# cvjena/ITAL

Hardware: AMD Instinct MI355X
Metric: MI-scored candidates/sec per fetch_unlabelled(k) round (higher is better)
Workload: dtype f64; 1 GPU; USPS-shaped synthetic 9298x256, k=4, perfect user, full 2^t enumeration, fetch_unlabelled + update per step; n=9298, d=256, k=4, parallelism=candidate rows sharded over 1 GPU(s), 1 record all-gather per greedy step

## Files before the change

include/ital_hip.h:

```cpp
#ifndef ITAL_HIP_H
#define ITAL_HIP_H

#include <stdint.h>

#ifdef __cplusplus
extern "C" {
#endif

typedef struct ihipStream_t* hipStream_t;

#define ITAL_MAX_T 8
#define ITAL_REC_HEADER 10
#define ITAL_JUMP_BITS 48
#define ITAL_GENERIC_MAX_DIM 20
#define ITAL_GENERIC_MAX_REL 16
#define ITAL_GENERIC_MAX_CALLS (1 << 22)
#define ITAL_TOPK_MAX 4096
#define ITAL_ROUND_MAX_CAND (1 << 21)

const char* ital_version(void);
const char* ital_last_error(void);
int64_t ital_launch_count(void);


int ital_row_norms(const double* X, int64_t n, int ldx, double* xnorm, hipStream_t stream);

int ital_rbf_cols(const double* X, const double* xnorm, int64_t n, int ldx, const double* Xs, const double* sn,
                  int c, double var, double length_scale, double* out, int64_t ldo, hipStream_t stream);

int ital_cross_cov_cols(const double* X, const double* xnorm, int64_t n, int ldx, const double* Xs,
                        const double* sn, int c, const double* W, int ldw, const double* V, int64_t ldv, int m,
                        double var, double length_scale, double* out, int64_t ldo, hipStream_t stream);

int ital_chol_append(const double* XT, const double* XTn, int ldx, double* L, int ldl, double* alpha,
                     const double* ynew, int m, int c, double var, double length_scale, double noise, int* status,
                     hipStream_t stream);

typedef struct ital_label_batch {
    int c;
    int slot[16];
    double y[16];
} ital_label_batch;
int ital_stage_labelled(const double* rows, int ldx, ital_label_batch lb, double* XT_dst, double* XTn_dst, double* y_dst,
                        hipStream_t stream);

typedef struct ital_append_desc {
    const double* rows;
    int ldx;
    ital_label_batch lb;
    const double* X;
    const double* xnorm;
    int64_t n;
    double* XT;
    double* XTn;
    double* L;
    int ldl;
    double* alpha;
    double* ybuf;
    double* V;
    int64_t ldv;
    int m;
    double var, length_scale, noise;
    double* mu;
    double* s2;
    int* status;
} ital_append_desc;
int ital_gp_append(const ital_append_desc* a, hipStream_t stream);

int ital_whiten_append(const double* X, const double* xnorm, int64_t n, int ldx, const double* Xnew,
                       const double* snew, int c, const double* L21, int ldw, const double* L22,
                       const double* alpha_new, double* V, int64_t ldv, int m, double var, double length_scale,
                       double* mu, double* s2, hipStream_t stream);

int ital_predict(const double* Xt, int64_t nt, int ldx, const double* XT, const double* XTn, int m, const double* L,
                 int ldl, const double* alpha, double var, double length_scale, double* mean, double* pvar, double* xtn,
                 double* Vt, int64_t ldvt, int clamp, hipStream_t stream);

int ital_topk(const double* v, int64_t n, int64_t index_offset, int k, double* out_vals, int64_t* out_idx, void* work,
              hipStream_t stream);
int64_t ital_topk_workspace(void);

int ital_mvn_seed(int state[6]);
int ital_mvn_draws_per_call(int n);
int ital_mvn_advance(int state[6], int64_t n_draws);
int ital_mvn_round_seeds(int state[6], int64_t n_cand, int k, int seeds[][6]);
int ital_mvn_tables(int t, long long* jump, long long* jumppat, double* vk);
int ital_mvn_generic_tables(int nmax, long long* jump1, double* vk_all);

// ... 233 lines not shown
```

ital_amd/_fast_round.py:

```python
import collections
import ctypes
import time

import numpy as np
import torch

from . import _lib, mvn_stream, sharding
from ._batch import (Scored, ensure_step_buffers, fill_score_desc, fill_score_select, lattice_label, lattice_tables)
from ._lib import check
from .gp import _ptr, _stream
from .retrieval_base import UnseenList

PREPARED, COMPACT, UPLOAD = "prepared", "compact", "upload"

DeviceList = collections.namedtuple("DeviceList", "buffers unseen version picks n_loc")


class Prepared(collections.namedtuple("Prepared", "desc slot k n n_loc m begin cur state_before state_after draws events sig")):
    __slots__ = ()

    def matches(self, k, n, m, stream_state, signature):
        return (self.k == k and self.n == n and self.m == m and self.state_before == tuple(stream_state)
                and self.sig == signature)

# ... 203 lines not shown

    def _download(self):
        L, k, hc = self.L, self.k, self.L.host_clock
        if hc is not None:
            hc["enqueue_s"] += time.perf_counter() - self.t_call
        host = L._download(self.rb.b["ret"], "the picks of the round", L._step_estimate_s(k, self.n_loc)).tolist()
        if hc is not None:
            hc["t_download"] = time.perf_counter()
        keep = self.keep
        L.last_scores = [keep[t, :self.n_loc] for t in range(k)] if keep is not None else []
        return host[:k], host[self.rb.b["kmax"]]

    def _finish(self, ret, status, saved_stream):
        L, gp, c = self.L, self.gp, self.candidates
        if status & 8:
            raise RuntimeError("ital_amd: the candidate list kept on the device lost track of the host's (internal error)")
        if status & 6:
            gp.status.bitwise_and_(~6)
            self.stream.state, self.stream.draws = saved_stream
            return L._fetch_generic(self.k, c.array() if self.listed else c)
        if status:
            gp.check_status(status)
        ret = [int(i) for i in ret]
        L._last_batch = (self.rb.b, list(ret))
        if self.listed:
            self.rb.device_list = DeviceList(self.rb, c, c.version, ret, self.n_loc)
        return ret
```

ital_amd/_lib.py:

```python
import ctypes
import os

HERE = os.path.dirname(os.path.abspath(__file__))
LIB_PATH = os.environ.get("ITAL_HIP_LIB", os.path.join(HERE, "libital_hip.so"))

c_void_p, c_int, c_int64, c_double = ctypes.c_void_p, ctypes.c_int, ctypes.c_int64, ctypes.c_double

ITAL_MAX_T = 8
ITAL_REC_HEADER = 10
ITAL_JUMP_BITS = 48
ITAL_GENERIC_MAX_DIM = 20
ITAL_GENERIC_MAX_REL = 16
ITAL_GENERIC_MAX_CALLS = 1 << 22
ITAL_TOPK_MAX = 4096
ITAL_ROUND_MAX_CAND = 1 << 21


class ItalBatch(ctypes.Structure):
    _fields_ = [("kmax", c_int), ("ldx", c_int), ("ldw", c_int), ("bidx", c_void_p), ("bgpos", c_void_p),
                ("bsort", c_void_p), ("bmu", c_void_p), ("sig", c_void_p), ("XB", c_void_p), ("XBn", c_void_p),
                ("VB", c_void_p)]


class ItalLabelBatch(ctypes.Structure):
    _fields_ = [("c", c_int), ("slot", c_int * 16), ("y", c_double * 16)]


class ItalAppendDesc(ctypes.Structure):
    _fields_ = [("rows", c_void_p), ("ldx", c_int), ("lb", ItalLabelBatch), ("X", c_void_p), ("xnorm", c_void_p), ("n", c_int64),
                ("XT", c_void_p), ("XTn", c_void_p), ("L", c_void_p), ("ldl", c_int), ("alpha", c_void_p), ("ybuf", c_void_p),
                ("V", c_void_p), ("ldv", c_int64), ("m", c_int), ("var", c_double), ("length_scale", c_double),
                ("noise", c_double), ("mu", c_void_p), ("s2", c_void_p), ("status", c_void_p)]


class ItalScoreDesc(ctypes.Structure):
    _fields_ = [("t", c_int), ("n_cand", c_int64), ("cand", c_void_p), ("alive", c_void_p), ("mu", c_void_p),
                ("s2", c_void_p), ("C", c_void_p), ("ldc", c_int64), ("row_offset", c_int64),
                ("pos_offset", c_int64), ("gpos", c_void_p), ("batch", ItalBatch), ("noise", c_double), ("eps", c_double),
                ("label_mode", c_int), ("mi", c_void_p), ("seed", c_int * 6), ("jump", c_void_p), ("jumppat", c_void_p),
                ("vk", c_void_p), ("status", c_void_p), ("work", c_void_p), ("work_doubles", c_int64), ("ev_start", c_void_p),
                ("ev_stop", c_void_p), ("sel_X", c_void_p), ("sel_xnorm", c_void_p), ("sel_ldx", c_int), ("sel_V", c_void_p),
                ("sel_ldv", c_int64), ("sel_m", c_int), ("sel_ldw", c_int), ("sel_rank", c_int), ("sel_record", c_void_p),
                ("sel_ret", c_void_p), ("sel_parts", c_void_p), ("sel_parts_len", c_int64), ("sel_counter", c_void_p)]


EXCHANGE_FN = ctypes.CFUNCTYPE(c_int, c_void_p, c_void_p, c_void_p, c_int, c_void_p)


class ItalRoundDesc(ctypes.Structure):
    _fields_ = [("k", c_int), ("step", ItalScoreDesc), ("seeds", (c_int * 6) * (ITAL_MAX_T + 1)),
                ("jump", c_void_p * (ITAL_MAX_T + 1)), ("jumppat", c_void_p * (ITAL_MAX_T + 1)),
                ("vk", c_void_p * (ITAL_MAX_T + 1)), ("ev_start", c_void_p * (ITAL_MAX_T + 1)),
                ("ev_stop", c_void_p * (ITAL_MAX_T + 1)), ("n_rows", c_int64), ("var", c_double), ("length_scale", c_double),
                ("mi_keep", c_void_p), ("begin", c_int), ("cand_prev", c_void_p), ("n_prev", c_int64),
                ("world", c_int), ("records_all", c_void_p), ("nccl_comm", c_void_p), ("exchange", EXCHANGE_FN),
# ... 29 lines not shown

class ItalNpLegacyState(ctypes.Structure):
    _fields_ = [("key", ctypes.c_uint32 * 624), ("pos", ctypes.c_int32), ("has_gauss", ctypes.c_int32), ("gauss", c_double)]


SIGNATURES = {
    "ital_version": (ctypes.c_char_p, []),
    "ital_mvn_seed": (c_int, [ctypes.POINTER(c_int)]),
    "ital_mvn_draws_per_call": (c_int, [c_int]),
    "ital_mvn_advance": (c_int, [ctypes.POINTER(c_int), c_int64]),
    "ital_mvn_round_seeds": (c_int, [ctypes.POINTER(c_int), c_int64, c_int, c_void_p]),
    "ital_mvn_tables": (c_int, [c_int, c_void_p, c_void_p, c_void_p]),
    "ital_mvn_generic_tables": (c_int, [c_int, c_void_p, c_void_p]),
    "ital_np_legacy_normals": (c_int, [ctypes.POINTER(ItalNpLegacyState), c_int64, c_void_p, c_int64, c_int]),
    "ital_last_error": (ctypes.c_char_p, []),
    "ital_launch_count": (c_int64, []),
    "ital_row_norms": (c_int, [c_void_p, c_int64, c_int, c_void_p, c_void_p]),
    "ital_rbf_cols": (c_int, [c_void_p, c_void_p, c_int64, c_int, c_void_p, c_void_p, c_int, c_double, c_double,
                              c_void_p, c_int64, c_void_p]),
    "ital_cross_cov_cols": (c_int, [c_void_p, c_void_p, c_int64, c_int, c_void_p, c_void_p, c_int, c_void_p, c_int,
                                    c_void_p, c_int64, c_int, c_double, c_double, c_void_p, c_int64, c_void_p]),
    "ital_chol_append": (c_int, [c_void_p, c_void_p, c_int, c_void_p, c_int, c_void_p, c_void_p, c_int, c_int,
                                 c_double, c_double, c_double, c_void_p, c_void_p]),
    "ital_whiten_append": (c_int, [c_void_p, c_void_p, c_int64, c_int, c_void_p, c_void_p, c_int, c_void_p, c_int,
                                   c_void_p, c_void_p, c_void_p, c_int64, c_int, c_double, c_double, c_void_p,
                                   c_void_p, c_void_p]),
    "ital_stage_labelled": (c_int, [c_void_p, c_int, ItalLabelBatch, c_void_p, c_void_p, c_void_p, c_void_p]),
    "ital_gp_append": (c_int, [ctypes.POINTER(ItalAppendDesc), c_void_p]),
    "ital_predict": (c_int, [c_void_p, c_int64, c_int, c_void_p, c_void_p, c_int, c_void_p, c_int, c_void_p,
                             c_double, c_double, c_void_p, c_void_p, c_void_p, c_void_p, c_int64, c_int, c_void_p]),
    "ital_topk": (c_int, [c_void_p, c_int64, c_int64, c_int, c_void_p, c_void_p, c_void_p, c_void_p]),
    "ital_topk_workspace": (c_int64, []),
    "ital_score_step": (c_int, [ctypes.POINTER(ItalScoreDesc), c_void_p]),
    "ital_score_workspace": (c_int64, [c_int, c_int64]),
    "ital_fetch_round": (c_int, [ctypes.POINTER(ItalRoundDesc), c_void_p]),
    "ital_cov_block": (c_int, [c_void_p, c_void_p, c_int64, c_void_p, c_void_p, c_int64, c_int, c_void_p, c_int64,
                               c_void_p, c_int64, c_int, c_double, c_double, c_void_p, c_int64, c_void_p]),
    "ital_cov_abs_rowsum": (c_int, [c_void_p, c_void_p, c_int64, c_void_p, c_void_p, c_int64, c_int, c_void_p, c_int64,
                                    c_void_p, c_int64, c_int, c_double, c_double, c_void_p, c_int64, c_int, c_void_p,
                                    c_void_p]),
    "ital_mcmi_score_step": (c_int, [ctypes.POINTER(ItalMcmiDesc), c_void_p]),
    "ital_mcmi_workspace": (c_int64, [c_int, c_int64]),
    "ital_score_generic": (c_int, [ctypes.POINTER(ItalGscoreDesc), c_void_p]),
    "ital_score_generic_workspace": (c_int64, [ctypes.POINTER(ItalGscoreDesc)]),
    "ital_select_local": (c_int, [c_void_p, c_void_p, c_void_p, c_int64, c_int64, c_void_p, c_int64, c_int, c_int, c_void_p,
                                  c_void_p, c_void_p, c_void_p, c_int, c_void_p, c_int64, c_int, c_int, c_void_p,
# ... 159 lines not shown
```

ital_amd/csrc/chol.hip:

```cpp
#include <hip/hip_runtime.h>
#include <stdint.h>

#include "device_math.h"
#include "ital_hip.h"
#include "ital_internal.h"

namespace ital {

__device__ __forceinline__ double readlane_f64(double v, int l) {
    return __hiloint2double(__builtin_amdgcn_readlane(__double2hiint(v), l), __builtin_amdgcn_readlane(__double2loint(v), l));
}

struct StageArgs {
    const double* rows;
    ital_label_batch lb;
    double* XT_w;
    double* XTn_w;
    double* y_w;
};

__global__ __launch_bounds__(1024) void chol_append_kernel(const double* XT, const double* XTn,
                                                           int ldx, double* __restrict__ L, int ldl,
                                                           double* __restrict__ alpha, const double* ynew,
                                                           int m, int c, double var, double s, double noise,
                                                           int* __restrict__ status, StageArgs sa) {
    __shared__ double S[16][17];
    __shared__ double tvec[16];
    __shared__ double Lb[64][65];
    const int lane = threadIdx.x & 63;
    const int j = threadIdx.x >> 6;
    const int g = m + j;
    double* Lg = L + (int64_t)g * ldl;
    if (sa.rows) {
        if (j < c) {
            const double* src = sa.rows + (int64_t)sa.lb.slot[j] * ldx;
            double* dst = sa.XT_w + (int64_t)j * ldx;
            double acc = 0;
            for (int k = lane; k < ldx; k += 64) {
                const double v = src[k];
                dst[k] = v;
                acc += v * v;
            }
            acc = wave_sum(acc);
            if (lane == 0) { sa.XTn_w[j] = acc; sa.y_w[j] = sa.lb.y[j]; }
        }
        __threadfence_block();
        __syncthreads();
    }
#ifdef ITAL_CHOL_TIMING
    long long tstamp[6];
    tstamp[0] = __builtin_readcyclecounter();
#define CHOL_STAMP(i) tstamp[i] = __builtin_readcyclecounter()
#else
#define CHOL_STAMP(i)
#endif
    {
        const int sub = threadIdx.x & 15;
        const int npair = (m + c) * c;
        for (int p0 = 0; p0 < npair; p0 += (int)blockDim.x >> 4) {
            const int pr = p0 + ((int)threadIdx.x >> 4);
            const bool live = pr < npair;
            const int jn = live ? pr % c : 0, r = live ? pr / c : 0;
            const int gn = m + jn;
            const bool need = live && r <= gn;
            double d0 = 0, d1 = 0;
            if (need) {
                const double* xa = XT + (int64_t)gn * ldx + 2 * sub;
                const double* xb = XT + (int64_t)r * ldx + 2 * sub;
                for (int k0 = 0; k0 < ldx; k0 += 256) {
                    double2 a[8], b[8];
#pragma unroll
                    for (int u = 0; u < 8; u++) {
                        const int k = k0 + 32 * u;
                        const bool in = k + 2 * sub < ldx;
                        a[u] = in ? *reinterpret_cast<const double2*>(xa + k) : double2{0, 0};
                        b[u] = in ? *reinterpret_cast<const double2*>(xb + k) : double2{0, 0};
                    }
#pragma unroll
                    for (int u = 0; u < 8; u++) {
                        d0 = fma(a[u].x, b[u].x, d0);
                        d1 = fma(a[u].y, b[u].y, d1);
                    }
                }
            }
            double dot = d0 + d1;
#pragma unroll
            for (int off = 1; off < 16; off <<= 1) dot += __shfl_xor(dot, off, 64);
            if (need && sub == 0) {
                double kv = var * exp((XTn[gn] + XTn[r] - 2 * dot) / s);
                if (r == gn) kv += noise;
                L[(int64_t)gn * ldl + r] = kv;
            }
        }
    }
    CHOL_STAMP(1);
    for (int r0 = 0; r0 < m; r0 += 64) {
        const int nb = m - r0 < 64 ? m - r0 : 64;
        __syncthreads();
        for (int idx = threadIdx.x; idx < nb * nb; idx += blockDim.x) {
            const int i = idx / nb, q = idx - i * nb;
            Lb[i][q] = L[(int64_t)(r0 + i) * ldl + r0 + q];
        }
        __syncthreads();
        if (j < c) {
            const bool in = lane < nb;
            double b = 0.0;
            if (in) {
                b = Lg[r0 + lane];
                const double* Li = L + (int64_t)(r0 + lane) * ldl;
                for (int q = 0; q < r0; q++) b = fma(-Li[q], Lg[q], b);
            }
            const double dinv = in ? 1.0 / Lb[lane][lane] : 1.0;
            double lq = Lb[lane][0];
            for (int q = 0; q < nb; q++) {
                const double lnext = Lb[lane][q + 1 < nb ? q + 1 : q];
                const double xq = readlane_f64(b * dinv, q);
                if (lane == q) b = xq;
                else if (lane > q && in) b = fma(-lq, xq, b);
// ... 53 lines not shown
            else if (mine && lane > q) tv -= S[lane][q] * xq;
        }
        if (mine) {
            for (int b = 0; b < c; b++) L[(int64_t)(m + lane) * ldl + m + b] = b <= lane ? S[lane][b] : 0.0;
            alpha[m + lane] = tv;
        }
        if (bad && lane == 0) atomicOr(status, 1);
    }
#ifdef ITAL_CHOL_TIMING
    CHOL_STAMP(4);
    if (threadIdx.x == 0)
        for (int i = 0; i < 4; i++) alpha[ldl - 8 + i] = (double)(tstamp[i + 1] - tstamp[i]);
#endif
}

}

extern "C" int ital_chol_append(const double* XT, const double* XTn, int ldx, double* L, int ldl, double* alpha,
                                const double* ynew, int m, int c, double var, double length_scale, double noise,
                                int* status, hipStream_t stream) {
    if (c < 1 || c > 16) return ital_fail(-22, "ital_chol_append: c must be in 1..16");
    if (m < 0 || m + c > ldl) return ital_fail(-22, "ital_chol_append: factor capacity exceeded");
    ITAL_LAUNCH(ital::chol_append_kernel, dim3(1), dim3(1024), 0, stream, XT, XTn, ldx, L, ldl, alpha, ynew, m,
                       c, var, -2.0 * length_scale * length_scale, noise, status, ital::StageArgs{});
    return ital_check_launch("ital_chol_append");
}

extern "C" int ital_gp_append(const ital_append_desc* a, hipStream_t stream) {
    if (!a) return ital_fail(-22, "ital_gp_append: null descriptor");
    const int c = a->lb.c, m = a->m;
    if (c < 1 || c > 16) return ital_fail(-22, "ital_gp_append: 1..16 samples per call");
    if (m < 0 || m + c > a->ldl) return ital_fail(-22, "ital_gp_append: factor capacity exceeded");
    if (a->ldx % 16 != 0) return ital_fail(-22, "ital_gp_append: ldx must be a multiple of 16");
    ital::StageArgs sa = {a->rows, a->lb, a->XT + (int64_t)m * a->ldx, a->XTn + m, a->ybuf};
    ITAL_LAUNCH(ital::chol_append_kernel, dim3(1), dim3(1024), 0, stream, a->XT, a->XTn, a->ldx, a->L, a->ldl, a->alpha,
                a->ybuf, m, c, a->var, -2.0 * a->length_scale * a->length_scale, a->noise, a->status, sa);
    const int rc = ital_check_launch("ital_gp_append(chol)");
    if (rc) return rc;
    const double* L21 = a->L + (int64_t)m * a->ldl;
    return ital_whiten_append(a->X, a->xnorm, a->n, a->ldx, a->XT + (int64_t)m * a->ldx, a->XTn + m, c, L21, a->ldl, L21 + m,
                              a->alpha + m, a->V, a->ldv, m, a->var, a->length_scale, a->mu, a->s2, stream);
}
```

ital_amd/gp.py:

```python
import ctypes
import os
import time

import numpy as np
import torch

from . import _lib, sharding
from ._lib import check


def _pad16(v):
    return (int(v) + 15) // 16 * 16


def _ptr(t):
    return 0 if t is None else t.data_ptr()


def _stream():
    return torch.cuda.current_stream().cuda_stream


def appends_after_remove(appends, p):
    out = list(appends)
    at = 0
    for g, c in enumerate(out):
        if at <= p < at + abs(c):
            if c < 0:
                raise ValueError("labelled position %d is a query" % p)
            out[g] = c - 1
            return out
        at += abs(c)
    raise ValueError("labelled position %d outside the %d labelled samples" % (p, at))


class GaussianProcess(object):

    def __init__(self, data, length_scale, var=1.0, noise=1e-6, pdist=None, *, device=None, rank=0, world=1,
                 group=None, capacity=None):
        if pdist is not None:
            raise NotImplementedError("pre-computed distances are a dense-kernel feature of the reference (gp.py:116-128)")
        if not torch.cuda.is_available():
            raise RuntimeError("ital_amd.GaussianProcess needs a HIP device (no CPU fallback)")
        self._lib = _lib.lib()
        self.device = torch.device(device if device is not None else "cuda:0")
        self.rank, self.world, self.group = int(rank), int(world), group
        self.collective = self.world > 1 or (group is not None and os.environ.get("ITAL_FORCE_COLLECTIVES") == "1")
        local = None
        if isinstance(data, sharding.ShardedRows):
            local = data
        else:
            data = np.asarray(data, dtype=np.float64)
        if data.ndim != 2:
            raise ValueError("data must be an n-by-d array")
        self.n_total, self.d = data.shape
        self.row0, self.row1 = sharding.row_range(self.n_total, self.world, self.rank)
        if local is not None and (local.row0, local.row1) != (self.row0, self.row1):
            raise ValueError("ShardedRows holds rows [%d, %d), this rank owns [%d, %d)"
                             % (local.row0, local.row1, self.row0, self.row1))
        self.n = self.row1 - self.row0
        self.ldx = _pad16(self.d)
        self.ldv = _pad16(max(self.n, 1))
        self.length_scale = length_scale
        self.length_scale_sq = length_scale * length_scale
        self.var = var
        self.noise = noise
        self.X_host = data
# ... 8 lines not shown
            self.status = torch.zeros(1, dtype=torch.int32, device=self.device)
            self._gather_bufs = {}
            if capacity is None:
                capacity = int(min(256, max(64, (2 << 30) // (8 * self.ldv))))
            self._alloc(capacity)
        self.reset()

    def _alloc(self, cap):
        cap = _pad16(cap)
        dev = self.device
        old = getattr(self, "cap", 0)
        V = torch.zeros((cap, self.ldv), dtype=torch.float64, device=dev)
        L = torch.zeros((cap, cap), dtype=torch.float64, device=dev)
        alpha = torch.zeros(cap, dtype=torch.float64, device=dev)
        XT = torch.zeros((cap, self.ldx), dtype=torch.float64, device=dev)
        XTn = torch.zeros(cap, dtype=torch.float64, device=dev)
        if old:
            V[:old] = self.V
            L[:old, :old] = self.L
            alpha[:old] = self.alpha
            XT[:old] = self.XT
            XTn[:old] = self.XTn
        self.V, self.L, self.alpha, self.XT, self.XTn, self.cap = V, L, alpha, XT, XTn, cap

    @property
    def X(self):
        return self.X_host

    @property
    def K_all(self):
        raise AttributeError("the dense N x N kernel matrix is never formed by ital_amd (reference gp.py:128 is "
                             "replaced by column streaming); use rbf_cols()")

    def _factor(self):
        return self.L[: self.m, : self.m].cpu().numpy()

    @property
    def K(self):
        if self.m == 0:
            return None
        f = self._factor()
        return f @ f.T

    @property
    def K_inv(self):
        if self.m == 0:
# ... 14 lines not shown
                raise RuntimeError("the GP has not been fitted")
            a, b = self.XT[: self.m, : self.d].cpu().numpy(), a
        a = np.atleast_2d(np.asarray(a, dtype=np.float64))
        b = np.atleast_2d(np.asarray(b, dtype=np.float64))
        dev = self.device
        A = torch.zeros((len(a), self.ldx), dtype=torch.float64, device=dev)
        B = torch.zeros((len(b), self.ldx), dtype=torch.float64, device=dev)
        A[:, : self.d] = torch.from_numpy(np.ascontiguousarray(a)).to(dev)
        B[:, : self.d] = torch.from_numpy(np.ascontiguousarray(b)).to(dev)
        an = torch.empty(len(a), dtype=torch.float64, device=dev)
        bn = torch.empty(len(b), dtype=torch.float64, device=dev)
        out = torch.empty((len(a), _pad16(len(b))), dtype=torch.float64, device=dev)
        st = _stream()
        check(self._lib.ital_row_norms(_ptr(A), len(a), self.ldx, _ptr(an), st))
        check(self._lib.ital_row_norms(_ptr(B), len(b), self.ldx, _ptr(bn), st))
        check(self._lib.ital_cov_block(_ptr(A), _ptr(an), len(a), _ptr(B), _ptr(bn), len(b), self.ldx, 0, 0, 0, 0, 0,
                                       float(self.var), float(self.length_scale), _ptr(out), out.shape[1], st))
        return out[:, : len(b)].cpu().numpy()

    def reset(self):
        self.ind = []
        self.y = None
        self.m = 0
        self.appends = []
        self.mu = torch.zeros(max(self.n, 1), dtype=torch.float64, device=self.device)
        self.s2 = torch.full((max(self.n, 1),), float(self.var), dtype=torch.float64, device=self.device)
        self.mu_all = torch.zeros(self.n_total, dtype=torch.float64, device=self.device) if self.collective else self.mu[: self.n]
        self._mean_host = None
        self.status.zero_()

    def fit(self, ind, y):
        self.reset()
        return self.update(ind, y)

    def update(self, ind, y, row_cache=None):
        ind = [int(i) for i in ind]
        y = np.asarray(y, dtype=np.float64).reshape(-1)
        if len(ind) != len(y):
            raise ValueError("ind and y differ in length")
        if len(ind) == 0:
            return self
        hc = getattr(self, "host_clock", None)
        t0 = time.perf_counter() if hc is not None else 0.0
        if row_cache is not None and all(i in row_cache[1] for i in ind):
            if len(ind) <= 16:
                self._append_staged(row_cache[0], [row_cache[1][i] for i in ind], y)
            else:
                slots = torch.as_tensor([row_cache[1][i] for i in ind], dtype=torch.int64, device=self.device)
                self._append(row_cache[0].index_select(0, slots), y)
        else:
            self._append(self._gather_rows(ind), y)
        self.ind += ind
        self.y = y.copy() if self.y is None else np.concatenate((self.y, y))
        self.appends.append(len(ind))
        t1 = time.perf_counter() if hc is not None else 0.0
        self._replicate_mean()
        if hc is not None:
            hc["append_s"] = hc.get("append_s", 0.0) + (t1 - t0)
            hc["means_s"] = hc.get("means_s", 0.0) + (time.perf_counter() - t1)
        return self

    def update_points(self, points, y, ind=None):
        pts = np.atleast_2d(np.asarray(points, dtype=np.float64))
        y = np.asarray(y, dtype=np.float64).reshape(-1)
        rows = torch.zeros((len(pts), self.ldx), dtype=torch.float64, device=self.device)
        rows[:, : self.d] = torch.from_numpy(np.ascontiguousarray(pts)).to(self.device)
        self._append(rows, y)
        self.ind += list(ind) if ind is not None else list(range(self.n_total + self.m - len(y), self.n_total + self.m))
        self.y = y.copy() if self.y is None else np.concatenate((self.y, y))
        self.appends.append(-len(y))
        self._replicate_mean()
        return self

    def _owned(self, ind):
# ... 5 lines not shown

    def _gather_rows(self, ind):
        if not self.collective:
            idx = torch.as_tensor(ind, dtype=torch.int64, device=self.device)
            return self.Xd.index_select(0, idx)
        mask, loc, any_own = self._owned(ind)
        if any_own:
            rows = self.Xd.index_select(0, loc) * mask[:, None]
        else:
            rows = torch.zeros((len(ind), self.ldx), dtype=torch.float64, device=self.device)
        sharding.all_reduce_sum(rows, self.group)
        return rows

    def gather_columns(self, mat, ind):
        mask, loc, any_own = self._owned(ind)
        if any_own:
            out = mat.index_select(1, loc) * mask[None, :]
        else:
            out = torch.zeros((mat.shape[0], len(loc)), dtype=torch.float64, device=self.device)
        if self.collective:
            sharding.all_reduce_sum(out, self.group)
        return out

    def _append_staged(self, matrix, slots, y):
        c = len(slots)
        if self.m + c > self.cap:
            self._alloc(max(2 * self.cap, self.m + c))
        if getattr(self, "_ybuf", None) is None:
            self._ybuf = torch.empty(16, dtype=torch.float64, device=self.device)
        d = getattr(self, "_append_desc", None)
        key = (self.V.data_ptr(), self.mu.data_ptr(), self.cap)
        if d is None or d[0] != key:
            a = _lib.ItalAppendDesc()
            a.ldx, a.X, a.xnorm, a.n = self.ldx, _ptr(self.Xd), _ptr(self.xnorm), self.n
            a.XT, a.XTn, a.L, a.ldl, a.alpha, a.ybuf = _ptr(self.XT), _ptr(self.XTn), _ptr(self.L), self.cap, _ptr(self.alpha), \
                _ptr(self._ybuf)
            a.V, a.ldv, a.mu, a.s2, a.status = _ptr(self.V), self.ldv, _ptr(self.mu), _ptr(self.s2), _ptr(self.status)
            self._append_desc = d = (key, a)
        a = d[1]
        a.rows, a.m = _ptr(matrix), self.m
        a.var, a.length_scale, a.noise = float(self.var), float(self.length_scale), float(self.noise)
        a.lb.c = c
        for j in range(c):
            a.lb.slot[j] = int(slots[j])
            a.lb.y[j] = float(y[j])
        check(self._lib.ital_gp_append(ctypes.byref(a), _stream()))
        self.m += c

    def _append(self, rows, y):
        lib, st = self._lib, _stream()
        c_total = rows.shape[0]
        if self.m + c_total > self.cap:
            self._alloc(max(2 * self.cap, self.m + c_total))
        yd = torch.from_numpy(np.ascontiguousarray(y)).to(self.device)
        for c0 in range(0, c_total, 16):
            c = min(16, c_total - c0)
            m = self.m
            self.XT[m:m + c] = rows[c0:c0 + c]
            check(lib.ital_row_norms(_ptr(self.XT[m:m + c]), c, self.ldx, _ptr(self.XTn[m:m + c]), st))
            check(lib.ital_chol_append(_ptr(self.XT), _ptr(self.XTn), self.ldx, _ptr(self.L), self.cap, _ptr(self.alpha),
                                       _ptr(yd[c0:c0 + c]), m, c, float(self.var), float(self.length_scale),
                                       float(self.noise), _ptr(self.status), st))
            L21 = self.L[m:]
            check(lib.ital_whiten_append(_ptr(self.Xd), _ptr(self.xnorm), self.n, self.ldx, _ptr(self.XT[m:m + c]),
                                         _ptr(self.XTn[m:m + c]), c, _ptr(L21), self.cap,
                                         L21.data_ptr() + 8 * m, _ptr(self.alpha[m:m + c]), _ptr(self.V), self.ldv, m,
                                         float(self.var), float(self.length_scale), _ptr(self.mu), _ptr(self.s2), st))
            self.m += c

    def remove(self, ind):
        ind = [int(i) for i in ind]
        if not ind:
            return self
        if len(set(ind)) != len(ind):
            raise ValueError("a sample is named twice")
        pos_of = {i: p for p, i in enumerate(self.ind)}
        for i in ind:
            if i >= self.n_total:
                raise ValueError("%d is a query row: queries cannot be removed" % i)
            if i not in pos_of:
                raise ValueError("sample %d has no label" % i)
        lib, st = self._lib, _stream()
        need = int(lib.ital_gp_remove_workspace(self.cap))
        work = getattr(self, "_remove_work", None)
        if work is None or work.numel() < need:
            self._remove_work = work = torch.empty(need, dtype=torch.float64, device=self.device)
        r = _lib.ItalRemoveDesc()
        r.XT, r.XTn, r.ldx, r.L, r.ldl, r.alpha = _ptr(self.XT), _ptr(self.XTn), self.ldx, _ptr(self.L), self.cap, _ptr(self.alpha)
        r.V, r.ldv, r.n, r.mu, r.s2 = _ptr(self.V), self.ldv, self.n, _ptr(self.mu), _ptr(self.s2)
        r.work, r.work_doubles, r.status = _ptr(work), work.numel(), _ptr(self.status)
        for p in sorted((pos_of[i] for i in ind), reverse=True):
            r.m, r.p = self.m, p
            check(lib.ital_gp_remove(ctypes.byref(r), st))
            self.appends = appends_after_remove(self.appends, p)
            del self.ind[p]
            self.y = np.delete(self.y, p)
            self.m -= 1
        if self.m == 0:
            self.reset()
        self._replicate_mean()
        return self

    def _whiten_rows(self, row_start, n_rows):
        r = _lib.ItalRewhitenDesc()
        r.X, r.n_rows, r.ldx = self.Xd.data_ptr() + 8 * row_start * self.ldx, n_rows, self.ldx
        r.XT, r.XTn, r.L, r.ldl, r.alpha, r.m = _ptr(self.XT), _ptr(self.XTn), _ptr(self.L), self.cap, _ptr(self.alpha), self.m
        r.var, r.length_scale = float(self.var), float(self.length_scale)
        r.xnorm, r.V, r.ldv, r.v_rows = self.xnorm.data_ptr() + 8 * row_start, self.V.data_ptr() + 8 * row_start, self.ldv, self.cap
        r.mu, r.s2, r.chunk = self.mu.data_ptr() + 8 * row_start, self.s2.data_ptr() + 8 * row_start, 0
        check(self._lib.ital_whiten_rows(ctypes.byref(r), _stream()))

    def extend(self, rows):
        rows = np.asarray(rows, dtype=np.float64)
# ... 4 lines not shown
        if self.world > 1 or not isinstance(self.X_host, np.ndarray):
            raise NotImplementedError("row sharding cannot grow yet: extend() needs all rows on one rank")
        k, n_old, m, dev = len(rows), self.n, self.m, self.device
        n_new = n_old + k
        ldv = _pad16(n_new)
        with torch.cuda.device(dev):
            Xd = torch.zeros((n_new, self.ldx), dtype=torch.float64, device=dev)
            Xd[:n_old] = self.Xd[:n_old]
            Xd[n_old:, : self.d] = torch.from_numpy(np.ascontiguousarray(rows)).to(dev)
            xnorm = torch.empty(n_new, dtype=torch.float64, device=dev)
            mu = torch.empty(n_new, dtype=torch.float64, device=dev)
            s2 = torch.empty(n_new, dtype=torch.float64, device=dev)
            V = torch.zeros((self.cap, ldv), dtype=torch.float64, device=dev)
            xnorm[:n_old], mu[:n_old], s2[:n_old] = self.xnorm[:n_old], self.mu[:n_old], self.s2[:n_old]
            if m and n_old:
                V[:m, :n_old] = self.V[:m, :n_old]
            self.Xd, self.xnorm, self.mu, self.s2, self.V = Xd, xnorm, mu, s2, V
            self.n, self.ldv = n_new, ldv
            self.ind = [i + k if i >= self.n_total else i for i in self.ind]
            self.n_total += k
            self.row1 = self.row0 + n_new
            self.X_host = np.concatenate((self.X_host, rows))
            self._append_desc = None
            self._gather_bufs = {}
            self._whiten_rows(n_old, k)
            self._replicate_mean()
        return self

    def set_params(self, length_scale=None, var=None, noise=None):
        ls = float(self.length_scale if length_scale is None else length_scale)
        var = float(self.var if var is None else var)
        noise = float(self.noise if noise is None else noise)
        if not (ls > 0 and var > 0):
            raise ValueError("length_scale and var must be positive")
        with torch.cuda.device(self.device):
            if self.m == 0:
                self.s2.fill_(var)
            else:
                lib, st, m = self._lib, _stream(), self.m
                L = torch.zeros((self.cap, self.cap), dtype=torch.float64, device=self.device)
                alpha = torch.zeros(self.cap, dtype=torch.float64, device=self.device)
                status = torch.zeros(1, dtype=torch.int32, device=self.device)
                yd = torch.from_numpy(np.ascontiguousarray(self.y, dtype=np.float64)).to(self.device)
                for c0 in range(0, m, 16):
                    c = min(16, m - c0)
                    check(lib.ital_chol_append(_ptr(self.XT), _ptr(self.XTn), self.ldx, _ptr(L), self.cap, _ptr(alpha),
                                               _ptr(yd[c0:c0 + c]), c0, c, var, ls, noise, _ptr(status), st))
                self.check_status(int(status.item()))
                self.L, self.alpha = L, alpha
                self._append_desc = None
            self.length_scale, self.length_scale_sq, self.var, self.noise = ls, ls * ls, var, noise
            if self.m:
                self._whiten_rows(0, self.n)
                self._replicate_mean()
        return self

    def evidence_chunk(self, max_bytes=1 << 30):
        m = self.m
        per = 8 * (m * m + int(self._lib.ital_gp_evidence_workspace(m, 1)) + 2 * m + 4)
        if per > max_bytes:
            raise MemoryError("one candidate at m = %d takes %d bytes, more than max_bytes = %d" % (m, per, max_bytes))
        return int(min(max_bytes // per, 65535))

    def evidence(self, params_list, *, max_bytes=1 << 30, events=None):
        if self.m == 0:
            raise RuntimeError("the GP has not been fitted")
        prm = np.empty((len(params_list), 3), dtype=np.float64)
        for g, p in enumerate(params_list):
            unknown = set(p) - {"length_scale", "var", "noise"}
            if unknown:
                raise TypeError("unexpected GP parameters: %s" % ", ".join(sorted(unknown)))
            prm[g] = (float(p.get("length_scale", self.length_scale)), float(p.get("var", self.var)),
                      float(p.get("noise", self.noise)))
            if not (prm[g, 0] > 0 and prm[g, 1] > 0):
# ... 188 lines not shown
```

ital_amd/ital.py:

```python
import ctypes
import os

import numpy as np
import torch

from . import _lib, _mc_sampler, mvn_stream, sharding
from ._lib import ITAL_GENERIC_MAX_CALLS, ITAL_GENERIC_MAX_DIM, ITAL_GENERIC_MAX_REL, ITAL_MAX_T, ItalScoreDesc, check
from ._batch import (FUSED_LAUNCH_MAX as _FUSED_LAUNCH_MAX, LABEL_MODES as _LABEL_MODES, Scored, ensure_step_buffers,
                     fill_score_desc, fill_score_select, gp_model, lattice_label, lattice_tables, make_batch_buffers,
                     member_column, qmc_work, select_step)
from ._fast_round import FastRound
from ._generic_round import GenericRound
from ._mc_sampler import range_cuts as _range_cuts
from .gp import _ptr, _stream
from .retrieval_base import ActiveRetrievalBase, UnseenList

_FUSED_SELECT_MAX = _lib.ITAL_ROUND_MAX_CAND


class ITAL(ActiveRetrievalBase):

    def __init__(self, data=None, queries=[], length_scale=0.1, var=1.0, noise=1e-6, label_prob=1.0,
                 mistake_prob=0.0, top_candidates=None, change_estimation_subset=0, clip_cov=0,
                 label_estimation='mean', monte_carlo_num_rel=None, monte_carlo_num_fb=None, parallelized=True, *,
# ... 247 lines not shown
                ev0 = self._mark() if t < 3 else None
                check(lib.ital_score_step(ctypes.byref(desc), st))
                if t < 3:
                    self._mark("score", t, n_alive, ev0)
                if self.keep_scores:
                    self.last_scores.append(mi.clone())
                if not (tail and fused):
                    select_step(gp, b, scored, gp_model(gp), t - 1, st, fused=fused, local=not tail, mark=self._mark)
                if t < k:
                    ev0 = self._mark() if t == 1 else None
                    member_column(self, gp_model(gp), b, t - 1, st)
                    if t == 1:
                        self._mark("cross_cov", t, gp.m, ev0)
                stream.advance(mvn_stream.step_draws(t, n_alive))
                n_alive -= 1
            host = self._download(b["ret"], "the picks of the round", self._step_estimate_s(k, n_loc)).tolist()
            ret, status = host[:k], host[b["kmax"]]
            if status & 6:
                gp.status.bitwise_and_(~6)
                stream.state, stream.draws = saved_stream
                return self._fetch_generic(k, candidates)
        if status:
            gp.check_status(status)
        self._last_batch = (b, list(ret))
        return [int(i) for i in ret]

    def _round_possible(self, k, candidates):
        gp = self.gp
        n = len(candidates)
        if n < k:
            return False
        if not gp.collective:
            return n <= _FUSED_SELECT_MAX
        if not isinstance(candidates, UnseenList) or self._round_transport() is None:
            return False
        bounds = [sharding.row_range(gp.n_total, gp.world, r)[0] for r in range(gp.world)] + [gp.n_total]
        sizes = np.diff([candidates.count_below(x) for x in bounds])
        return bool(sizes.min() >= 1 and sizes.max() <= _FUSED_SELECT_MAX)

    @staticmethod
    def _step_estimate_s(k, n_loc):
        if k < 3:
            return 0.0
        prime = (31, 47, 73, 113, 173, 263, 397, 593, 907, 1361)[min(k - 1, 10) - 1]
        return float(n_loc) * (2 ** k) * 16 * prime * (k - 1) / 1e11

    def _download(self, tensor, what, step_estimate_s=0.0):
# ... 43 lines not shown
```

ital_amd/mcmi.py:

```python
import collections
import ctypes

import numpy as np
import torch

from . import _lib, sharding
from ._batch import FUSED_LAUNCH_MAX, Model, Scored, make_batch_buffers, member_column, select_step
from ._lib import ITAL_MAX_T, ItalMcmiDesc, check
from .gp import _pad16, _ptr, _stream
from .retrieval_base import ActiveRetrievalBase


BlockBufs = collections.namedtuple("BlockBufs", "key X V vec")
FetchBufs = collections.namedtuple("FetchBufs", "key b cov pos alive ce")


class MCMI_min(ActiveRetrievalBase):

    max_cov_bytes = 96 << 30

    def __init__(self, data=None, queries=[], length_scale=0.1, var=1.0, noise=1e-6, subsample=None,
                 parallelized=True, *, device=None, rank=0, world=1, group=None):
        ActiveRetrievalBase.__init__(self, data, queries, length_scale, var, noise, device=device, rank=rank,
                                     world=world, group=group)
# ... 113 lines not shown
                                     float(self.length_scale), _ptr(fb.cov), ldc, st))
        self._mark("cov_block", 0, nc, ev0)
        self.last_scores = []
        for t in range(1, k + 1):
            desc = ItalMcmiDesc()
            desc.t = t
            self._fill_desc(desc, fb, scored, block, nc)
            if t >= 5 and n_i:
                self._workspace(desc, b, t, n_i)
            ev0 = self._mark()
            check(lib.ital_mcmi_score_step(ctypes.byref(desc), st))
            self._mark("mcmi_score", t, nc - (t - 1), ev0)
            if self.keep_scores:
                self.last_scores.append(scored.scores.clone())
            select_step(gp, b, scored, block, t - 1, st, argmin=1, fused=not gp.collective and n_i <= FUSED_LAUNCH_MAX)
            if t < k:
                member_column(self, block, b, t - 1, st)

    def _finish(self, k, cand, b):
        host = b["ret"].cpu().tolist()
        picked = host[:k]
        self.gp.check_status(host[b["kmax"]])
        ret = [int(cand[p]) for p in picked]
        self._last_batch = (b, ret)
        self._candidates = (cand, picked)
        return ret

    def fetch_unlabelled(self, k, show_progress=False):
        gp = self.gp
        if gp.m == 0:
            raise RuntimeError("fetch_unlabelled() needs a fitted relevance model: call update() first or pass queries")
        cand = self._unseen_array()
        if self.subsample and (self.subsample < len(cand)):
            cand = np.random.choice(cand, self.subsample, replace=False)
        if len(cand) < k:
            k = len(cand)
        if k <= 0:
            self.candidates = cand.tolist()
            return []
        if k > ITAL_MAX_T:
            raise NotImplementedError("batches larger than %d are not enumerated on the device" % ITAL_MAX_T)
        self._last_batch = None
        cand = np.asarray(cand, dtype=np.int64)
        nc = len(cand)
        with torch.cuda.device(gp.device):
            st = _stream()
            Xc, Vc, ldc, xnc, muc, s2c = self._gather_block(cand)
# ... 15 lines not shown
```

ital_amd/retrieval_base.py:

```python
import numpy as np

from . import tune
from .gp import GaussianProcess


class IdSet(set):

    _serial = 0

    def __init__(self, *a):
        set.__init__(self, *a)
        IdSet._serial += 1 << 20
        self.changes = IdSet._serial


def _counting(name):
    base = getattr(set, name)

    def method(self, *a, **kw):
        self.changes += 1
        return base(self, *a, **kw)
    method.__name__ = name
    method.__doc__ = base.__doc__
    return method
# ... 260 lines not shown
    def tune_params(self, grid=tune.default_grids['ls_only'], criterion='lml', apply=True, verbose=0):
        best, score = tune.optimize_session_params(self, grid, criterion=criterion, verbose=verbose)
        if score == -np.inf:
            raise np.linalg.LinAlgError("no candidate of the grid has a positive definite kernel matrix of the labelled samples")
        if apply:
            self.set_params(**best)
        return best, score

    def relabel(self, feedback):
        changed = []
        for i, fb in feedback.items():
            old = 1 if i in self.relevant_ids else -1 if i in self.irrelevant_ids else 0 if i in self.unnameable_ids else None
            new = 1 if fb > 0 else -1 if fb < 0 else 0
            if old is not None and old != new:
                changed.append(i)
        if changed:
            self.revoke(changed)
        self.update(feedback)

    def _batch_rows(self):
        last = getattr(self, "_last_batch", None)
        if not last:
            return None
        b, picks = last
        return b["XB"], {int(i): slot for slot, i in enumerate(picks)}

    def updated_prediction(self, feedback, test_ind, cov_mode='full'):
        rel, irr, _ = self.partition_feedback(feedback)
        if len(rel) + len(irr) == 0:
            return self.gp.predict_stored(test_ind, cov_mode=cov_mode)
        rel.sort()
        irr.sort()
        return self.gp.updated_prediction(rel + irr, np.concatenate((np.ones(len(rel)), -1 * np.ones(len(irr)))),
                                          test_ind, cov_mode=cov_mode)

    def partition_feedback(self, feedback):
        rel, irr, unnameable = [], [], []
        for i, fb in feedback.items():
            if fb > 0:
                if i in self.irrelevant_ids:
                    raise RuntimeError('Cannot change feedback once given.')
                elif i not in self.relevant_ids:
                    rel.append(i)
            elif fb < 0:
                if i in self.relevant_ids:
                    raise RuntimeError('Cannot change feedback once given.')
                elif i not in self.irrelevant_ids:
                    irr.append(i)
# ... 4 lines not shown
```

Before: 15.98 million candidates/s.

## Reuse whitened candidate columns from the batch to skip triangular solve in append

```diff
diff --git a/include/ital_hip.h b/include/ital_hip.h
--- a/include/ital_hip.h
+++ b/include/ital_hip.h
@@ -35,6 +35,10 @@
 int ital_chol_append(const double* XT, const double* XTn, int ldx, double* L, int ldl, double* alpha,
                      const double* ynew, int m, int c, double var, double length_scale, double noise, int* status,
                      hipStream_t stream);
+
+int ital_chol_append_cols(const double* XT, const double* XTn, int ldx, double* L, int ldl, double* alpha,
+                          const double* ynew, int m, int c, double var, double length_scale, double noise,
+                          const double* vcols, int ldvc, const int* slots, int* status, hipStream_t stream);
 
 typedef struct ital_label_batch {
     int c;
@@ -64,6 +68,9 @@
     double* mu;
     double* s2;
     int* status;
+    const double* vcols;
+    int ldvc;
+    int m_cols;
 } ital_append_desc;
 int ital_gp_append(const ital_append_desc* a, hipStream_t stream);
 
diff --git a/ital_amd/_fast_round.py b/ital_amd/_fast_round.py
--- a/ital_amd/_fast_round.py
+++ b/ital_amd/_fast_round.py
@@ -249,7 +249,7 @@
         if status:
             gp.check_status(status)
         ret = [int(i) for i in ret]
-        L._last_batch = (self.rb.b, list(ret))
+        L._last_batch = (self.rb.b, list(ret), (self.p.m, gp.factor_gen))
         if self.listed:
             self.rb.device_list = DeviceList(self.rb, c, c.version, ret, self.n_loc)
         return ret
diff --git a/ital_amd/_lib.py b/ital_amd/_lib.py
--- a/ital_amd/_lib.py
+++ b/ital_amd/_lib.py
@@ -30,7 +30,8 @@
     _fields_ = [("rows", c_void_p), ("ldx", c_int), ("lb", ItalLabelBatch), ("X", c_void_p), ("xnorm", c_void_p), ("n", c_int64),
                 ("XT", c_void_p), ("XTn", c_void_p), ("L", c_void_p), ("ldl", c_int), ("alpha", c_void_p), ("ybuf", c_void_p),
                 ("V", c_void_p), ("ldv", c_int64), ("m", c_int), ("var", c_double), ("length_scale", c_double),
-                ("noise", c_double), ("mu", c_void_p), ("s2", c_void_p), ("status", c_void_p)]
+                ("noise", c_double), ("mu", c_void_p), ("s2", c_void_p), ("status", c_void_p), ("vcols", c_void_p),
+                ("ldvc", c_int), ("m_cols", c_int)]
 
 
 class ItalScoreDesc(ctypes.Structure):
@@ -106,6 +107,9 @@
                                     c_void_p, c_int64, c_int, c_double, c_double, c_void_p, c_int64, c_void_p]),
     "ital_chol_append": (c_int, [c_void_p, c_void_p, c_int, c_void_p, c_int, c_void_p, c_void_p, c_int, c_int,
                                  c_double, c_double, c_double, c_void_p, c_void_p]),
+    "ital_chol_append_cols": (c_int, [c_void_p, c_void_p, c_int, c_void_p, c_int, c_void_p, c_void_p, c_int, c_int,
+                                      c_double, c_double, c_double, c_void_p, c_int, ctypes.POINTER(c_int), c_void_p,
+                                      c_void_p]),
     "ital_whiten_append": (c_int, [c_void_p, c_void_p, c_int64, c_int, c_void_p, c_void_p, c_int, c_void_p, c_int,
                                    c_void_p, c_void_p, c_void_p, c_int64, c_int, c_double, c_double, c_void_p,
                                    c_void_p, c_void_p]),
diff --git a/ital_amd/csrc/chol.hip b/ital_amd/csrc/chol.hip
--- a/ital_amd/csrc/chol.hip
+++ b/ital_amd/csrc/chol.hip
@@ -19,11 +19,17 @@
     double* y_w;
 };
 
+struct ColArgs {
+    const double* cols;
+    int ld;
+    int slot[16];
+};
+
 __global__ __launch_bounds__(1024) void chol_append_kernel(const double* XT, const double* XTn,
                                                            int ldx, double* __restrict__ L, int ldl,
                                                            double* __restrict__ alpha, const double* ynew,
                                                            int m, int c, double var, double s, double noise,
-                                                           int* __restrict__ status, StageArgs sa) {
+                                                           int* __restrict__ status, StageArgs sa, ColArgs ca) {
     __shared__ double S[16][17];
     __shared__ double tvec[16];
     __shared__ double Lb[64][65];
@@ -56,11 +62,12 @@
 #endif
     {
         const int sub = threadIdx.x & 15;
-        const int npair = (m + c) * c;
+        const int r_first = ca.cols ? m : 0;
+        const int npair = (m + c - r_first) * c;
         for (int p0 = 0; p0 < npair; p0 += (int)blockDim.x >> 4) {
             const int pr = p0 + ((int)threadIdx.x >> 4);
             const bool live = pr < npair;
-            const int jn = live ? pr % c : 0, r = live ? pr / c : 0;
+            const int jn = live ? pr % c : 0, r = r_first + (live ? pr / c : 0);
             const int gn = m + jn;
             const bool need = live && r <= gn;
             double d0 = 0, d1 = 0;
@@ -94,6 +101,12 @@
         }
     }
     CHOL_STAMP(1);
+    if (ca.cols) {
+        if (j < c) {
+            const double* vc = ca.cols + (int64_t)ca.slot[j] * ca.ld;
+            for (int r = lane; r < m; r += 64) Lg[r] = vc[r];
+        }
+    } else
     for (int r0 = 0; r0 < m; r0 += 64) {
         const int nb = m - r0 < 64 ? m - r0 : 64;
         __syncthreads();
@@ -193,8 +206,26 @@
     if (c < 1 || c > 16) return ital_fail(-22, "ital_chol_append: c must be in 1..16");
     if (m < 0 || m + c > ldl) return ital_fail(-22, "ital_chol_append: factor capacity exceeded");
     ITAL_LAUNCH(ital::chol_append_kernel, dim3(1), dim3(1024), 0, stream, XT, XTn, ldx, L, ldl, alpha, ynew, m,
-                       c, var, -2.0 * length_scale * length_scale, noise, status, ital::StageArgs{});
+                       c, var, -2.0 * length_scale * length_scale, noise, status, ital::StageArgs{}, ital::ColArgs{});
     return ital_check_launch("ital_chol_append");
+}
+
+extern "C" int ital_chol_append_cols(const double* XT, const double* XTn, int ldx, double* L, int ldl, double* alpha,
+                                     const double* ynew, int m, int c, double var, double length_scale, double noise,
+                                     const double* vcols, int ldvc, const int* slots, int* status, hipStream_t stream) {
+    if (c < 1 || c > 16) return ital_fail(-22, "ital_chol_append_cols: c must be in 1..16");
+    if (m < 0 || m + c > ldl) return ital_fail(-22, "ital_chol_append_cols: factor capacity exceeded");
+    if (!vcols) return ital_fail(-22, "ital_chol_append_cols: no whitened columns (ital_chol_append solves for them)");
+    if (ldvc < m) return ital_fail(-22, "ital_chol_append_cols: ldvc is smaller than m");
+    ital::ColArgs ca = {vcols, ldvc, {0}};
+    for (int j = 0; j < c; j++) {
+        ca.slot[j] = slots ? slots[j] : j;
+        if (ca.slot[j] < 0) return ital_fail(-22, "ital_chol_append_cols: negative slot");
+    }
+    if (m == 0) ca.cols = nullptr;
+    ITAL_LAUNCH(ital::chol_append_kernel, dim3(1), dim3(1024), 0, stream, XT, XTn, ldx, L, ldl, alpha, ynew, m,
+                       c, var, -2.0 * length_scale * length_scale, noise, status, ital::StageArgs{}, ca);
+    return ital_check_launch("ital_chol_append_cols");
 }
 
 extern "C" int ital_gp_append(const ital_append_desc* a, hipStream_t stream) {
@@ -203,9 +234,19 @@
     if (c < 1 || c > 16) return ital_fail(-22, "ital_gp_append: 1..16 samples per call");
     if (m < 0 || m + c > a->ldl) return ital_fail(-22, "ital_gp_append: factor capacity exceeded");
     if (a->ldx % 16 != 0) return ital_fail(-22, "ital_gp_append: ldx must be a multiple of 16");
+    ital::ColArgs ca = {};
+    if (a->vcols) {
+        if (a->m_cols != m) return ital_fail(-22, "ital_gp_append: the whitened columns were gathered at another m (m_cols != m)");
+        if (a->ldvc < m) return ital_fail(-22, "ital_gp_append: ldvc is smaller than m");
+        if (m > 0) {
+            ca.cols = a->vcols;
+            ca.ld = a->ldvc;
+            for (int j = 0; j < c; j++) ca.slot[j] = a->lb.slot[j];
+        }
+    }
     ital::StageArgs sa = {a->rows, a->lb, a->XT + (int64_t)m * a->ldx, a->XTn + m, a->ybuf};
     ITAL_LAUNCH(ital::chol_append_kernel, dim3(1), dim3(1024), 0, stream, a->XT, a->XTn, a->ldx, a->L, a->ldl, a->alpha,
-                a->ybuf, m, c, a->var, -2.0 * a->length_scale * a->length_scale, a->noise, a->status, sa);
+                a->ybuf, m, c, a->var, -2.0 * a->length_scale * a->length_scale, a->noise, a->status, sa, ca);
     const int rc = ital_check_launch("ital_gp_append(chol)");
     if (rc) return rc;
     const double* L21 = a->L + (int64_t)m * a->ldl;
diff --git a/ital_amd/gp.py b/ital_amd/gp.py
--- a/ital_amd/gp.py
+++ b/ital_amd/gp.py
@@ -7,6 +7,9 @@
 
 from . import _lib, sharding
 from ._lib import check
+
+
+APPEND_FROM_COLUMNS = os.environ.get("ITAL_APPEND_FROM_COLUMNS", "1") != "0"
 
 
 def _pad16(v):
@@ -43,6 +46,9 @@
         if not torch.cuda.is_available():
             raise RuntimeError("ital_amd.GaussianProcess needs a HIP device (no CPU fallback)")
         self._lib = _lib.lib()
+        self.append_from_columns = APPEND_FROM_COLUMNS
+        self.factor_gen = 0
+        self.append_paths = {"batch_columns": 0, "gathered_columns": 0, "substitution": 0}
         self.device = torch.device(device if device is not None else "cuda:0")
         self.rank, self.world, self.group = int(rank), int(world), group
         self.collective = self.world > 1 or (group is not None and os.environ.get("ITAL_FORCE_COLLECTIVES") == "1")
@@ -97,6 +103,7 @@
             XT[:old] = self.XT
             XTn[:old] = self.XTn
         self.V, self.L, self.alpha, self.XT, self.XTn, self.cap = V, L, alpha, XT, XTn, cap
+        self.factor_gen += 1
 
     @property
     def X(self):
@@ -157,6 +164,7 @@
         self.ind = []
         self.y = None
         self.m = 0
+        self.factor_gen += 1
         self.appends = []
         self.mu = torch.zeros(max(self.n, 1), dtype=torch.float64, device=self.device)
         self.s2 = torch.full((max(self.n, 1),), float(self.var), dtype=torch.float64, device=self.device)
@@ -179,12 +187,14 @@
         t0 = time.perf_counter() if hc is not None else 0.0
         if row_cache is not None and all(i in row_cache[1] for i in ind):
             if len(ind) <= 16:
-                self._append_staged(row_cache[0], [row_cache[1][i] for i in ind], y)
+                cols = row_cache[2:4] if len(row_cache) >= 5 and self.columns_valid(row_cache[4]) else None
+                self._append_staged(row_cache[0], [row_cache[1][i] for i in ind], y, cols)
             else:
                 slots = torch.as_tensor([row_cache[1][i] for i in ind], dtype=torch.int64, device=self.device)
                 self._append(row_cache[0].index_select(0, slots), y)
         else:
-            self._append(self._gather_rows(ind), y)
+            own = not self.collective and all(0 <= i < self.n for i in ind)
+            self._append(self._gather_rows(ind), y, col_ids=ind if own else None)
         self.ind += ind
         self.y = y.copy() if self.y is None else np.concatenate((self.y, y))
         self.appends.append(len(ind))
@@ -236,7 +246,16 @@
             sharding.all_reduce_sum(out, self.group)
         return out
 
-    def _append_staged(self, matrix, slots, y):
+    def batch_state(self):
+        return (self.m, self.factor_gen)
+
+    APPEND_COLS_MIN_M = 1
+
+    def columns_valid(self, state):
+        return (self.append_from_columns and state is not None and tuple(state) == self.batch_state()
+                and self.m >= self.APPEND_COLS_MIN_M)
+
+    def _append_staged(self, matrix, slots, y, cols=None):
         c = len(slots)
         if self.m + c > self.cap:
             self._alloc(max(2 * self.cap, self.m + c))
@@ -253,6 +272,11 @@
             self._append_desc = d = (key, a)
         a = d[1]
         a.rows, a.m = _ptr(matrix), self.m
+        if cols is not None:
+            a.vcols, a.ldvc, a.m_cols = _ptr(cols[0]), int(cols[1]), self.m
+        else:
+            a.vcols, a.ldvc, a.m_cols = None, 0, 0
+        self.append_paths["batch_columns" if cols is not None else "substitution"] += 1
         a.var, a.length_scale, a.noise = float(self.var), float(self.length_scale), float(self.noise)
         a.lb.c = c
         for j in range(c):
@@ -261,7 +285,7 @@
         check(self._lib.ital_gp_append(ctypes.byref(a), _stream()))
         self.m += c
 
-    def _append(self, rows, y):
+    def _append(self, rows, y, col_ids=None):
         lib, st = self._lib, _stream()
         c_total = rows.shape[0]
         if self.m + c_total > self.cap:
@@ -272,9 +296,19 @@
             m = self.m
             self.XT[m:m + c] = rows[c0:c0 + c]
             check(lib.ital_row_norms(_ptr(self.XT[m:m + c]), c, self.ldx, _ptr(self.XTn[m:m + c]), st))
-            check(lib.ital_chol_append(_ptr(self.XT), _ptr(self.XTn), self.ldx, _ptr(self.L), self.cap, _ptr(self.alpha),
-                                       _ptr(yd[c0:c0 + c]), m, c, float(self.var), float(self.length_scale),
-                                       float(self.noise), _ptr(self.status), st))
+            if col_ids is not None and self.append_from_columns and m >= self.APPEND_COLS_MIN_M:
+                idx = torch.as_tensor(col_ids[c0:c0 + c], dtype=torch.int64, device=self.device)
+                vc = self.V[:m].index_select(1, idx).t().contiguous()
+                check(lib.ital_chol_append_cols(_ptr(self.XT), _ptr(self.XTn), self.ldx, _ptr(self.L), self.cap,
+                                                _ptr(self.alpha), _ptr(yd[c0:c0 + c]), m, c, float(self.var),
+                                                float(self.length_scale), float(self.noise), _ptr(vc), m, None,
+                                                _ptr(self.status), st))
+                self.append_paths["gathered_columns"] += 1
+            else:
+                check(lib.ital_chol_append(_ptr(self.XT), _ptr(self.XTn), self.ldx, _ptr(self.L), self.cap, _ptr(self.alpha),
+                                           _ptr(yd[c0:c0 + c]), m, c, float(self.var), float(self.length_scale),
+                                           float(self.noise), _ptr(self.status), st))
+                self.append_paths["substitution"] += 1
             L21 = self.L[m:]
             check(lib.ital_whiten_append(_ptr(self.Xd), _ptr(self.xnorm), self.n, self.ldx, _ptr(self.XT[m:m + c]),
                                          _ptr(self.XTn[m:m + c]), c, _ptr(L21), self.cap,
@@ -303,6 +337,7 @@
         r.XT, r.XTn, r.ldx, r.L, r.ldl, r.alpha = _ptr(self.XT), _ptr(self.XTn), self.ldx, _ptr(self.L), self.cap, _ptr(self.alpha)
         r.V, r.ldv, r.n, r.mu, r.s2 = _ptr(self.V), self.ldv, self.n, _ptr(self.mu), _ptr(self.s2)
         r.work, r.work_doubles, r.status = _ptr(work), work.numel(), _ptr(self.status)
+        self.factor_gen += 1
         for p in sorted((pos_of[i] for i in ind), reverse=True):
             r.m, r.p = self.m, p
             check(lib.ital_gp_remove(ctypes.byref(r), st))
@@ -353,6 +388,7 @@
             self.row1 = self.row0 + n_new
             self.X_host = np.concatenate((self.X_host, rows))
             self._append_desc = None
+            self.factor_gen += 1
             self._gather_bufs = {}
             self._whiten_rows(n_old, k)
             self._replicate_mean()
@@ -381,6 +417,7 @@
                 self.L, self.alpha = L, alpha
                 self._append_desc = None
             self.length_scale, self.length_scale_sq, self.var, self.noise = ls, ls * ls, var, noise
+            self.factor_gen += 1
             if self.m:
                 self._whiten_rows(0, self.n)
                 self._replicate_mean()
diff --git a/ital_amd/ital.py b/ital_amd/ital.py
--- a/ital_amd/ital.py
+++ b/ital_amd/ital.py
@@ -293,7 +293,7 @@
                 return self._fetch_generic(k, candidates)
         if status:
             gp.check_status(status)
-        self._last_batch = (b, list(ret))
+        self._last_batch = (b, list(ret), gp.batch_state())
         return [int(i) for i in ret]
 
     def _round_possible(self, k, candidates):
diff --git a/ital_amd/mcmi.py b/ital_amd/mcmi.py
--- a/ital_amd/mcmi.py
+++ b/ital_amd/mcmi.py
@@ -159,7 +159,7 @@
         picked = host[:k]
         self.gp.check_status(host[b["kmax"]])
         ret = [int(cand[p]) for p in picked]
-        self._last_batch = (b, ret)
+        self._last_batch = (b, ret, self.gp.batch_state())
         self._candidates = (cand, picked)
         return ret
 
diff --git a/ital_amd/retrieval_base.py b/ital_amd/retrieval_base.py
--- a/ital_amd/retrieval_base.py
+++ b/ital_amd/retrieval_base.py
@@ -306,8 +306,11 @@
         last = getattr(self, "_last_batch", None)
         if not last:
             return None
-        b, picks = last
-        return b["XB"], {int(i): slot for slot, i in enumerate(picks)}
+        b, picks = last[0], last[1]
+        slots = {int(i): slot for slot, i in enumerate(picks)}
+        if len(last) < 3 or last[2] is None:
+            return b["XB"], slots
+        return b["XB"], slots, b["VB"], b["ldw"], last[2]
 
     def updated_prediction(self, feedback, test_ind, cov_mode='full'):
         rel, irr, _ = self.partition_feedback(feedback)
```

After: 16.06 million candidates/s (median of 4 runs). No clear change (+0.5%).
